# hsinnan75/MapCaller

Hardware: AMD Instinct MI355X
Metric: reads/sec (150 bp PE vs GRCh38) at 1/2/4/8 MI355X; SAM CIGAR bit-exact (higher is better)
Workload: dtype u64/int32; 1 GPU; synthetic GRCh38-sized genome, 3100 Mbp (synthetic: GRCh38 is unavailable offline; repeat landscape in the detail record), 4000000 pairs x 150 bp PE per step per GPU (sub 0.005, ins 0.001, del 0.001 per base), -alg ksw2

## Files before the change

mapcaller_amd/csrc/mcx_glue.h:

```cpp
#ifndef MCX_GLUE_H
#define MCX_GLUE_H
#include "mcx_fm.h"

namespace mcx {

struct Ctx {
    IndexView ix;
    Params pm;
    Caps caps;
    Layout lay;
    uint8_t *detail;
    DetailLayout dlay;
    uint8_t *state;
    const uint8_t *mapq_tab;
    int32_t mapq_rows;
    uint32_t *cig_pool;
    uint32_t *cig_pool_n;
    uint32_t cig_pool_cap;
    const uint32_t *packed;
    int32_t wpad;
    const uint32_t *read_ext;
    int32_t dp_summary;
    const Hit *seed_pool;
};

constexpr int kCigStage = 4;

static inline MCX_HD int64_t hit_pd(const Hit &h) { return h.gPos - h.rPos; }

static inline MCX_HD int prep_seeds(Hit *h, int n)
{
    int m = 0;
    bool in_order = true;
    int64_t ppd = 0;
    int prp = 0;
    for (int i = 0; i < n; i++) {
        const Hit x = h[i];
        const int64_t pd = hit_pd(x);
        if (pd > 0) {
            if (m > 0 && (ppd > pd || (ppd == pd && prp > x.rPos))) in_order = false;
            if (m != i) h[m] = x;
            m++; ppd = pd; prp = x.rPos;
        }
    }
    if (in_order) return m;
    for (int gap = m > 24 ? (m > 400 ? 109 : 23) : 1; gap >= 1; gap = gap > 23 ? 23 : (gap > 5 ? 5 : (gap > 1 ? 1 : 0))) {
        for (int i = gap; i < m; i++) {
            const Hit key = h[i];
            const int64_t kpd = hit_pd(key);
            int j = i - gap;
            while (j >= 0) {
                const Hit y = h[j];
                const int64_t pd = hit_pd(y);
                if (pd > kpd || (pd == kpd && y.rPos > key.rPos)) { h[j + gap] = y; j -= gap; } else break;
            }
            if (j + gap != i) h[j + gap] = key;
        }
    }
    return m;
}

static inline MCX_HD int64_t boundary_of(const IndexView &ix, int64_t gPos)
{
    int s = end_slot(ix, gPos);
    return s < 0 ? -1 : ix.end_pos[s];
}

static inline MCX_HD void cand_init(Cand &dst, int score, int first, int count, int64_t pd0)
{
    Cand c;
    c.score = score; c.mate = -1; c.first = first; c.count = count; c.pd0 = pd0;
    c.frag_off = 0; c.n_frags = 0; c.flag = 0; c.fwd = 1; c.in_pool = 0; c.pad = 0; c.pool_off = 0;
    dst = c;
}

template <class Emit>
static inline MCX_HD int cluster_seeds_to(const IndexView &ix, const Params &pm, int rlen, const Hit *h, int n, Emit emit)
{
    if (n == 0) return 0;
    const Hit h0 = h[0];
    int nc = 0, head = 0, score = h0.len, thr = rlen >> 2;
    int64_t g_end = boundary_of(ix, h0.gPos);
    int64_t pd_prev = hit_pd(h0);
    for (int j = 1; j <= n; j++) {
        Hit hj; hj.gPos = ix.G2; hj.rPos = 0; hj.len = 0;
        if (j < n) hj = h[j];
        const int64_t gj = hj.gPos, pdj = j < n ? hit_pd(hj) : ix.G2;
        int64_t d = pdj - pd_prev;
        pd_prev = pdj;
        if (d < 0) d = -d;
        if (gj > g_end || d > pm.max_pos_diff) {
            if (score > thr) {
                if (thr < (score >> 1)) thr = score >> 1;
                int b = head, e = j, s = score;
                if (score >= rlen) {
                    int run_b = head, rs = h[head].len;
                    s = 0; b = e = head;
                    int k;
                    for (k = head + 1; k < j; k++) {
                        if (hit_pd(h[k]) != hit_pd(h[run_b])) {
                            if (rs > s) { s = rs; b = run_b; e = k; }
                            run_b = k; rs = h[k].len;
                        } else rs += h[k].len;
                    }
                    if (rs > s) { s = rs; b = run_b; e = k; }
                }
                emit(nc, s, b, e - b, hit_pd(h[b]));
                nc++;
            }
            head = j;
            if (j < n) { g_end = boundary_of(ix, gj); score = hj.len; }
        } else score += hj.len;
    }
    return nc;
}

static inline MCX_HD int cluster_seeds(const IndexView &ix, const Params &pm, int rlen, const Hit *h, int n,
                                       Cand *out, int cap)
{
    return cluster_seeds_to(ix, pm, rlen, h, n, [&](int k, int score, int first, int count, int64_t pd0) { if (k < cap) cand_init(out[k], score, first, count, pd0); });
}

static inline MCX_HD void keep_top_scores(Cand *c, int n)
{
    if (n <= 1) return;
    int best = 0;
    for (int i = 0; i < n; i++) if (c[i].score > best) best = c[i].score;
    for (int i = 0; i < n; i++) if (c[i].score < best) c[i].score = 0;
}

static inline MCX_HD int pair_by_distance(int64_t est, Cand *c1, int n1, Cand *c2, int n2, int &lo, int &hi)
{
    int64_t max_lt = -1, min_ge = 0x7fffffff;
    if (n1 * n2 > 100) { keep_top_scores(c1, n1); keep_top_scores(c2, n2); }
    int j0 = 0;
    auto partner = [&](const Cand &a, int &ps) {
        int pick = -1;
        ps = 0;
        while (j0 < n2 && c2[j0].pd0 < a.pd0) j0++;
        for (int j = j0; j < n2; j++) {
            const int sj = c2[j].score;
            if (sj == 0) continue;
            const int64_t d = c2[j].pd0 - a.pd0;
            if (d < est) {
                if (d > max_lt) max_lt = d;
                if (sj > ps) { pick = j; ps = sj; }
            } else { if (d < min_ge) min_ge = d; break; }
        }
        return pick;
    };
    int64_t top = 0;
    for (int i = 0; i < n1; i++) {
        const Cand a = c1[i];
        if (a.score == 0) continue;
        int ps;
        if (partner(a, ps) >= 0) { const int64_t s = (int64_t)a.score + ps; if (s > top) top = s; }
    }
    int paired = 0;
    if (top > 0) {
        j0 = 0;
        for (int i = 0; i < n1; i++) {
            const Cand a = c1[i];
            if (a.score == 0) continue;
            int ps;
            const int pick = partner(a, ps);
            if (pick >= 0 && (int64_t)a.score + ps == top) { paired++; c1[i].mate = pick; c2[pick].mate = i; }
        }
    }
    lo = (int)(max_lt + 1);
    hi = (int)min_ge;
    return paired;
}

static inline MCX_HD void mask_unpaired(Cand *c1, int n1, Cand *c2, int n2)
{
    int top = 0;
    for (int i = 0; i < n1; i++)
        if (c1[i].mate != -1 && top < c1[i].score + c2[c1[i].mate].score) top = c1[i].score + c2[c1[i].mate].score;
    for (int i = 0; i < n1; i++)
        if (c1[i].mate == -1 || c1[i].score + c2[c1[i].mate].score < top) c1[i].score = 0;
    for (int j = 0; j < n2; j++)
        if (c2[j].mate == -1 || c2[j].score + c1[c2[j].mate].score < top) c2[j].score = 0;
}

#define MCX_NOKMER 0xFFFFFFFFu

static inline MCX_HD uint8_t read_char(const ReadRef &r, int i)
{
    if (!r.flipped) return r.ascii[i];
    switch (r.ascii[r.rlen - 1 - i]) {
    case 'A': case 'a': return 'T';
    case 'C': case 'c': return 'G';
    case 'G': case 'g': return 'C';
    case 'T': case 't': return 'A';
    default: return 'N';
    }
}

template <class GetCh>
static inline MCX_HD void kmer_fill(GetCh ch, int len, uint32_t *out)
{
    for (int i = 0; i < len; i++) out[i] = MCX_NOKMER;
    uint32_t tail = 0, count = 0, head, wid;
    while (count < (uint32_t)kKmerSize && tail < (uint32_t)len) { if (ch(tail++) != 'N') count++; else count = 0; }
    if (count != (uint32_t)kKmerSize) return;
    head = tail - kKmerSize;
    wid = 0;
    for (uint32_t i = head; i < head + kKmerSize; i++) wid = (wid << 2) + (uint32_t)nt4_code(ch(i));
    out[head] = wid;
    for (head += 1; tail < (uint32_t)len; head++, tail++) {
        uint8_t c = ch(tail);
        if (c != 'N') {
            wid = ((wid & 0x3FFFu) << 2) + (uint32_t)nt4_code(c);
            out[head] = wid;
        } else {
            count = 0; tail++;
            while (count < (uint32_t)kKmerSize && tail < (uint32_t)len) { if (ch(tail++) != 'N') count++; else count = 0; }
            if (count != (uint32_t)kKmerSize) break;
            head = tail - kKmerSize;
            wid = 0;
            for (uint32_t i = head; i < head + kKmerSize; i++) wid = (wid << 2) + (uint32_t)nt4_code(ch(i));
            out[head] = wid;
        }
    }
}

struct RescueOut { int score; int n_seeds; int d; };

static inline MCX_HD int diag_scan(const uint32_t *kq, int qlen, const uint32_t *kg, int slen, int d, int64_t base,
                                   Hit *hits, int n_hits, int cap, int &emitted, bool &overflow)
{
    const int r0 = d < 0 ? -d : 0, r1 = qlen - 1 < slen - 1 - d ? qlen - 1 : slen - 1 - d;
    int total = 0, run = 0, run_start = 0;
    for (int r = r0; r <= r1 + 1; r++) {
        const bool m = r <= r1 && kq[r] != MCX_NOKMER && kq[r] == kg[r + d];
        if (m) { if (run == 0) run_start = r; run++; }
        else if (run > 0) {
            const int l = kKmerSize + run - 1;
            if (l >= 10) {
                total += l;
                if (hits) {
                    if (n_hits + emitted < cap) {
                        Hit h; h.rPos = run_start; h.gPos = (int64_t)(run_start + d) + base; h.len = l;
                        hits[n_hits + emitted] = h;
                    } else overflow = true;
                    emitted++;
                }
            }
            run = 0;
        }
    }
    return total;
}

static inline MCX_HD int diag_total(const uint32_t *kq, int qlen, const uint32_t *kg, int slen, int d)
{
    const int r0 = d < 0 ? -d : 0, r1 = qlen - 1 < slen - 1 - d ? qlen - 1 : slen - 1 - d;
    int total = 0;
    uint64_t hist = 0;
    for (int base = r0; base <= r1; base += 61) {
        uint64_t e = hist;
        const int n = r1 - base + 1 < 61 ? r1 - base + 1 : 61;
        for (int i = 0; i < n; i++) {
            const uint32_t q = kq[base + i];
            e |= (uint64_t)(q != MCX_NOKMER && q == kg[base + i + d]) << (3 + i);
        }
        const uint64_t t = e & (e >> 1) & (e >> 2);
        const uint64_t own = t & ~(uint64_t)1;
#if defined(__HIP_DEVICE_COMPILE__)
        total += __popcll(own) + 9 * __popcll(own & ~(t << 1));
#else
        total += __builtin_popcountll(own) + 9 * __builtin_popcountll(own & ~(t << 1));
#endif
        hist = (e >> 61) & 7u;
    }
    return total;
}

struct RescueSerial {
    uint32_t *kq, *kg;
    MCX_HD bool leader() const { return true; }
    MCX_HD void sync() const {}
    MCX_HD void fill_query(const ReadRef &rq) const
    {
        kmer_fill([&](uint32_t i) { return read_char(rq, (int)i); }, rq.rlen, kq);
    }
    MCX_HD RescueOut window(const IndexView &ix, int64_t left, int slen, int qlen, Hit *hits, int n_hits, int cap, bool &overflow) const
    {
        kmer_fill([&](uint32_t i) { return (uint8_t)"ACGT"[ref_code(ix, left + i)]; }, slen, kg);
        RescueOut best; best.score = 0; best.n_seeds = 0; best.d = 0;
        int dummy = 0;
        for (int d = -(qlen - 1); d <= slen - 1; d++) {
            const int total = diag_scan(kq, qlen, kg, slen, d, left, nullptr, 0, 0, dummy, overflow);
            if (total > best.score) { best.score = total; best.d = d; }
        }
        if (best.score > 0) diag_scan(kq, qlen, kg, slen, best.d, left, hits, n_hits, cap, best.n_seeds, overflow);
        return best;
    }
};

#if defined(__HIPCC__)
constexpr int kRescueQWords = 1024 / 32 + 2;
constexpr int rescue_wwords(int kg) { return (kg + 2 * 1056) / 32 + 4; }

static __device__ __forceinline__ uint32_t even_bits16(uint32_t t)
{
    t &= 0x55555555u; t = (t | (t >> 1)) & 0x33333333u; t = (t | (t >> 2)) & 0x0f0f0f0fu; t = (t | (t >> 4)) & 0x00ff00ffu;
    return (t | (t >> 8)) & 0xffffu;
}

struct RescueWave {
    uint32_t *q;
    uint32_t *w;
    uint32_t *ew;
    int wstride;
    int *red;
    uint32_t *kq, *kg;
    __device__ bool leader() const { return threadIdx.x == 0; }
    __device__ void sync() const { __threadfence_block(); __syncthreads(); }
    __device__ void fill_query(const ReadRef &rq) const
    {
        const int tid = threadIdx.x, nt = blockDim.x;
        uint32_t *ql = q, *qh = q + kRescueQWords, *qn = q + 2 * kRescueQWords;
        __syncthreads();
        for (int i = tid; i < 3 * kRescueQWords; i += nt) q[i] = 0u;
        if (tid == 0) red[0] = 0;
        __syncthreads();
        for (int i = tid; i < rq.rlen; i += nt) {
            const int c = nt4_code(read_char(rq, i));
            const uint32_t bit = 1u << (i & 31);
            if (c > 3) atomicOr(&qn[i >> 5], bit);
            else { if (c & 1) atomicOr(&ql[i >> 5], bit); if (c & 2) atomicOr(&qh[i >> 5], bit); }
        }
        __syncthreads();
        int any_n = 0;
        for (int k = tid; k < kRescueQWords; k += nt) any_n |= qn[k] != 0u;
        any_n = __syncthreads_or(any_n);
        if (tid == 0) red[2 * (nt >> 6) + 4] = any_n;
        if (any_n) {
            if (leader()) kmer_fill([&](uint32_t i) { return read_char(rq, (int)i); }, rq.rlen, kq);
            __threadfence_block();
            __syncthreads();
            return;
        }
        uint32_t v8 = 0;
        if (tid < kRescueQWords) {
            auto ok = [&](int k) -> uint32_t {
                if (k >= kRescueQWords || 32 * k >= rq.rlen) return 0u;
                const uint32_t in = rq.rlen - 32 * k >= 32 ? ~0u : ((1u << (rq.rlen - 32 * k)) - 1u);
                return ~qn[k] & in;
            };
            const uint32_t v = ok(tid), vn = ok(tid + 1);
            v8 = v;
#pragma unroll
            for (int j = 1; j < kKmerSize; j++) v8 &= __funnelshift_r(v, vn, j);
        }
        __syncthreads();
        if (tid < kRescueQWords) qn[tid] = v8;
        __syncthreads();
    }
    __device__ int diagonal(int d, int qlen, int slen, int pad, bool store) const
    {
        const uint32_t *ql = q, *qh = q + kRescueQWords, *qv = q + 2 * kRescueQWords, *wl = w, *wh = w + wstride;
        const int lo = d < 0 ? -d : 0, hi = qlen - kKmerSize < slen - kKmerSize - d ? qlen - kKmerSize : slen - kKmerSize - d;
        if (hi - lo < 2) return 0;
        const int ktop = (hi + kKmerSize - 1) >> 5, kbot = lo >> 5;
        const int s0 = d + pad, sh = s0 & 31;
        int i = ktop + (s0 >> 5);
        uint32_t wl_hi = wl[i + 1], wh_hi = wh[i + 1], m_hi = 0, a_hi = 0, b_hi = 0, e_hi = 0, t_hi = 0;
        int total = 0;
        for (int k = ktop; k >= kbot; k--, i--) {
            const uint32_t wl_lo = wl[i], wh_lo = wh[i];
            const uint32_t gl = __funnelshift_r(wl_lo, wl_hi, sh), gh = __funnelshift_r(wh_lo, wh_hi, sh);
            wl_hi = wl_lo; wh_hi = wh_lo;
            const uint32_t m = ~((ql[k] ^ gl) | (qh[k] ^ gh));
            const uint32_t a = m & __funnelshift_r(m, m_hi, 1);
            const uint32_t b = a & __funnelshift_r(a, a_hi, 2);
            const uint32_t c = b & __funnelshift_r(b, b_hi, 4);
            m_hi = m; a_hi = a; b_hi = b;
            const int x0 = lo - 32 * k, x1 = hi - 32 * k;
            const uint32_t rows = (x1 < 0 || x0 > 31) ? 0u : ((~0u << (x0 > 0 ? x0 : 0)) & (~0u >> (31 - (x1 < 31 ? x1 : 31))));
            const uint32_t e = c & qv[k] & rows;
            if (store) ew[k] = e;
            uint32_t t = 0;
            if (e | e_hi) {
                t = e & __funnelshift_r(e, e_hi, 1) & __funnelshift_r(e, e_hi, 2);
                total += __popc(t) + 9 * __popc(t & ~__funnelshift_r(t, t_hi, 1));
            }
            t_hi = t; e_hi = e;
        }
        return total;
    }
    __device__ RescueOut window_ids(const IndexView &ix, int64_t left, int slen, int qlen, Hit *hits, int n_hits, int cap, bool &overflow) const
    {
        const int tid = threadIdx.x, nt = blockDim.x, lane = tid & 63, wave = tid >> 6, n_waves = nt >> 6;
        __syncthreads();
        uint8_t *gb = (uint8_t *)(kg + slen + 8);
        if (left < ix.G && left + slen > ix.G) {
            for (int p = tid; p < slen; p += nt) {
                uint32_t wid = MCX_NOKMER;
                if (p + kKmerSize <= slen) { wid = 0; for (int k = 0; k < kKmerSize; k++) wid = (wid << 2) | (uint32_t)ref_code(ix, left + p + k); }
                kg[p] = wid;
            }
        } else {
        const bool rev = left >= ix.G;
        const int64_t f0 = rev ? ix.G2 - (left + slen) : left;
        const int64_t b0 = f0 >> 2;
        const int n_bytes = (int)(((f0 + slen - 1) >> 2) - b0) + 1;
        for (int i = tid; i < n_bytes; i += nt) gb[i] = ix.pac[b0 + i];
        __syncthreads();
        auto base = [&](int p) -> uint32_t {
            const int64_t f = rev ? f0 + (slen - 1 - p) : f0 + p;
            const uint32_t c = (gb[(f >> 2) - b0] >> ((~f & 3) << 1)) & 3u;
            return rev ? 3u - c : c;
        };
        for (int p = tid; p < slen; p += nt) {
            uint32_t wid = MCX_NOKMER;
// ... 891 lines not shown
```

mapcaller_amd/csrc/mcx_pipeline.hip:

```cpp
#include <hip/hip_runtime.h>
#include <algorithm>
#include <atomic>
#include <chrono>
#include <cmath>
#include <cstdio>
#include <cstdlib>
#include <cstring>
#include <string>
#include <type_traits>
#include <vector>

#include "../../include/mcx.h"
#include "mcx_dp.h"
#include "mcx_dp_lane2.h"
#include "mcx_simple.h"
#include "mcx_profile.h"
#include <hipcub/hipcub.hpp>
#include "mcx_internal.h"

using namespace mcx;

static thread_local std::string g_err;
static int fail(int code, const std::string &msg) { g_err = msg; return code; }
#define HIP_TRY(expr)                                                                         \
// ... 581 lines not shown
__global__ void __launch_bounds__(256) k_sa(Ctx cx, SeedOut so, int paired, uint32_t *lf_total)
{
    const uint32_t n = min(*so.n_tasks, so.task_cap);
    const int nr = paired ? 2 : 1;
    for (uint32_t t = blockIdx.x * blockDim.x + threadIdx.x; t < n; t += gridDim.x * blockDim.x) {
        const uint2 task = so.tasks[t];
        PairState st = pair_state(cx.state, cx.lay, cx.caps, task.x / nr);
        Hit &h = st.hits[task.x % nr][task.y];
        int lf = 0;
        h.gPos = (int64_t)fm_sa(cx.ix, (uint64_t)h.gPos, lf);
        if (lf_total && lf) atomicAdd(lf_total, (uint32_t)lf);
    }
}

struct RescueList { uint32_t *ids; uint32_t *n; uint32_t cap; };
struct EarlyList { uint32_t *ids; int32_t *est; uint32_t *n; uint32_t cap; uint32_t *n_hits; };

constexpr int kCntPad = 64;
constexpr int kWorkClasses = 6;
static __device__ __forceinline__ int work_class(uint32_t hits) { return hits > 64 ? 0 : hits > 32 ? 1 : hits > 16 ? 2 : hits > 8 ? 3 : hits > 4 ? 4 : 5; }

static __device__ __forceinline__ int pair_work_class(const PairSel &sel, uint32_t local, const uint32_t *read_blocks, int nr, const uint8_t *done = nullptr)
{
    if (done && done[local]) return -1;
    const uint32_t pair = sel_pair(sel, local);
    return work_class((read_blocks[pair * nr] >> 20) + (nr == 2 ? read_blocks[pair * nr + 1] >> 20 : 0u));
}

constexpr int kOrderTile = 16;

__global__ void __launch_bounds__(256) k_order_count(PairSel sel, const uint32_t *read_blocks, int nr, uint32_t *counts, const uint8_t *done)
{
    __shared__ uint32_t n_cls[kWorkClasses];
    if (threadIdx.x < kWorkClasses) n_cls[threadIdx.x] = 0u;
    __syncthreads();
    const uint32_t base = blockIdx.x * (256u * kOrderTile);
    for (int t = 0; t < kOrderTile; t++) {
        const uint32_t local = base + t * 256u + threadIdx.x;
        const int cls = local < sel.n ? pair_work_class(sel, local, read_blocks, nr, done) : -1;
#pragma unroll
        for (int k = 0; k < kWorkClasses; k++) {
            const uint64_t m = __ballot(cls == k);
            if ((threadIdx.x & 63) == 0 && m) atomicAdd(&n_cls[k], (uint32_t)__popcll(m));
        }
    }
    __syncthreads();
    if (threadIdx.x < kWorkClasses && n_cls[threadIdx.x]) atomicAdd(counts + threadIdx.x * kCntPad, n_cls[threadIdx.x]);
}

__global__ void __launch_bounds__(256) k_order_place(PairSel sel, const uint32_t *read_blocks, int nr, uint32_t *counts, uint32_t *order, const uint8_t *done)
{
    __shared__ uint32_t n_cls[kWorkClasses], at_cls[kWorkClasses];
    if (threadIdx.x < kWorkClasses) n_cls[threadIdx.x] = 0u;
    __syncthreads();
    const uint32_t base = blockIdx.x * (256u * kOrderTile);
    const int lane = threadIdx.x & 63;
    int cls[kOrderTile];
#pragma unroll
    for (int t = 0; t < kOrderTile; t++) {
        const uint32_t local = base + t * 256u + threadIdx.x;
        cls[t] = local < sel.n ? pair_work_class(sel, local, read_blocks, nr, done) : -1;
#pragma unroll
        for (int k = 0; k < kWorkClasses; k++) {
            const uint64_t m = __ballot(cls[t] == k);
            if (lane == 0 && m) atomicAdd(&n_cls[k], (uint32_t)__popcll(m));
        }
    }
    __syncthreads();
    if (threadIdx.x < kWorkClasses) {
        uint32_t first = 0;
        for (int k = 0; k < (int)threadIdx.x; k++) first += counts[k * kCntPad];
        const uint32_t mine = n_cls[threadIdx.x];
        at_cls[threadIdx.x] = first + (mine ? atomicAdd(counts + (8 + threadIdx.x) * kCntPad, mine) : 0u);
    }
    __syncthreads();
#pragma unroll
    for (int t = 0; t < kOrderTile; t++) {
        const uint32_t local = base + t * 256u + threadIdx.x;
#pragma unroll
        for (int k = 0; k < kWorkClasses; k++) {
            const uint64_t m = __ballot(cls[t] == k);
            uint32_t b = 0;
            if (lane == 0 && m) b = atomicAdd(&at_cls[k], (uint32_t)__popcll(m));
            b = __shfl(b, 0, 64);
            if (cls[t] == k) order[b + (uint32_t)__popcll(m & ((1ull << lane) - 1ull))] = local;
        }
    }
}

struct SimpleLater {
    uint32_t *pairs;
    SimpleJob *jobs;
    SimpleRes *res;
    uint32_t *job_list;
    uint32_t *n_pairs, *n_jobs;
    uint32_t cap;
};

template <bool NW, int MODE, bool DETAIL>
__global__ void __launch_bounds__(256) k_simple(Ctx cx, ReadBatch rb, uint32_t n_pairs, const int32_t *est, const uint32_t *read_blocks, AlnRec *recs, PairOut *pout,
                                                uint8_t *done, uint32_t *pool_over, uint32_t *n_done, SimpleLater sl)
{
    __shared__ EndsLds ends;
    __shared__ uint16_t cig_stage[256 * 2 * kSimpleRuns];
    __shared__ uint32_t job_stage[MODE == kDpCollect ? 3 * kSimpleJobs * 256 : 1];
    stage_ends(cx.ix, ends);
    const uint32_t slot = blockIdx.x * blockDim.x + threadIdx.x;
    const int nr = cx.pm.paired ? 2 : 1;
    uint16_t *stage = cig_stage + threadIdx.x;
    const uint32_t n_slots = MODE == kDpReplay ? min(*sl.n_pairs, sl.cap) : n_pairs;
    bool ok = slot < n_slots;
    const uint32_t pair = MODE == kDpReplay ? (ok ? sl.pairs[slot] : 0u) : slot;
    SimpleRead sr[2];
    int rl[2] = {0, 0};
    typename std::conditional<DETAIL, SimpleDetail, SimpleNoDetail>::type det;
    SimpleDpIo io;
    io.mode = MODE == kDpCollect && !sl.pairs ? kDpNone : MODE;
    io.jobs = MODE == kDpCollect ? job_stage + threadIdx.x : nullptr; io.job_stride = 256;
    io.res = MODE == kDpReplay ? sl.res + (uint64_t)slot * kSimpleJobs : nullptr;
    io.n = 0; io.read = 0;
    bool later = false;
    if (ok) {
        const PairState st = pair_state(cx.state, cx.lay, cx.caps, pair);
#pragma unroll
        for (int s = 0; s < 2; s++) {
            if (s < nr && ok) {
                const uint32_t r = pair * nr + s;
                const int nh = (int)(read_blocks[r] >> 20);
                rl[s] = (int)(rb.off[r + 1] - rb.off[r]);
                io.read = r;
                ok = nh >= 1 && nh <= kSimpleHits && !(cx.read_ext[r] >> 31);
                if (ok) {
                    if constexpr (DETAIL) { uint8_t *rec = cx.detail + (uint64_t)r * cx.dlay.stride; det.frags = (Frag *)(rec + sizeof(DetailHdr)); det.ops = rec + cx.dlay.off_ops; }
                    const int how = simple_read<NW, uint16_t>(cx.ix, cx.pm, rl[s], cx.packed + (uint64_t)r * cx.wpad, st.hits[s], nh, sr[s], stage + s * kSimpleRuns * 256, 256, io, det);
                    ok = how != kSimpleNo;
                    later = later || how == kSimpleLater;
                }
            }
        }
        if (ok && nr == 2) ok = simple_pair_ok(sr[0], sr[1], est[pair]);
    }
    if (MODE == kDpCollect) {
        const bool wait = ok && later;
        const uint32_t at = wave_reserve(sl.n_pairs, wait ? 1u : 0u);
        const bool kept = wait && at < sl.cap;
        const uint32_t jat = wave_reserve(sl.n_jobs, kept ? (uint32_t)io.n : 0u);
        if (kept) {
            sl.pairs[at] = pair;
            for (int k = 0; k < io.n; k++) {
                const uint32_t *w = job_stage + (3 * k) * 256 + threadIdx.x;
                sl.jobs[(uint64_t)at * kSimpleJobs + k] = simple_job_unpack(w[0], w[256], w[512], pair * (uint32_t)nr, nr);
                sl.job_list[jat + k] = at * kSimpleJobs + (uint32_t)k;
            }
            done[pair] = 2;
        }
        if (wait) ok = false;
        later = kept;
    }
    const uint32_t want = ok ? (uint32_t)sr[0].n_cig + (nr == 2 ? (uint32_t)sr[1].n_cig : 0u) : 0u;
    const uint32_t at = wave_reserve(cx.cig_pool_n, want);
    const uint64_t took = __ballot(ok);
    if ((threadIdx.x & 63) == 0 && took) atomicAdd(n_done, (uint32_t)__popcll(took));
    if (slot >= n_slots) return;
    if (ok && at + want > cx.cig_pool_cap) { atomicOr(pool_over, 1u); ok = false; }
    if (!later) done[pair] = ok ? 1 : 0;
    if (!ok) return;
    const uint32_t off[2] = {at, at + (uint32_t)sr[0].n_cig};
#pragma unroll
    for (int s = 0; s < 2; s++) {
        if (s >= nr) break;
        for (int k = 0; k < sr[s].n_cig; k++) cx.cig_pool[off[s] + k] = (uint32_t)stage[(s * kSimpleRuns + k) * 256];
    }
    AlnRec rec2[2];
    PairOut po;
    simple_pair(cx, nr == 2, sr[0], sr[nr - 1], rl[0], rl[nr - 1], est[pair], rec2, off, po);
    recs[(uint64_t)pair * nr] = rec2[0];
    if (nr == 2) recs[(uint64_t)pair * nr + 1] = rec2[1];
    pout[pair] = po;
    if constexpr (DETAIL) {
#pragma unroll
        for (int s = 0; s < 2; s++) {
            if (s >= nr) break;
            const DetailHdr d = simple_detail_hdr(cx.ix, nr == 2, s, sr[0], sr[nr - 1]);
            *(DetailHdr *)(cx.detail + ((uint64_t)pair * nr + s) * cx.dlay.stride) = d;
        }
    }
}

template <bool NW>
__global__ void __launch_bounds__(256) k_simple_dp(Ctx cx, SimpleLater sl)
{
    constexpr int W = 2 + kSimpleDp * LaneDir<16, NW>::words;
    __shared__ uint32_t words[W * 256];
    const uint32_t n = min(*sl.n_jobs, sl.cap * kSimpleJobs);
    LaneMem mem; mem.base = words; mem.stride = 256; mem.lane = threadIdx.x;
    for (uint32_t i = blockIdx.x * blockDim.x + threadIdx.x; i < n; i += gridDim.x * blockDim.x) {
        const uint32_t at = sl.job_list[i];
        const SimpleJob j = sl.jobs[at];
        sl.res[at] = simple_dp_job<NW>(cx.ix, j, cx.packed + (uint64_t)j.read * cx.wpad, mem);
    }
}

static __device__ __forceinline__ uint32_t listed_pairs(const PairSel &sel, const uint32_t *order_cnt)
{
    if (!order_cnt) return sel.n;
    uint32_t n = 0;
#pragma unroll
    for (int k = 0; k < kWorkClasses; k++) n += order_cnt[k * kCntPad];
    return n;
}

__global__ void __launch_bounds__(256) k_cluster(Ctx cx, ReadBatch rb, PairSel sel, RescueList rl, const uint32_t *read_blocks, EarlyList el, const uint32_t *order,
                                                 const uint32_t *order_cnt, int cls_lo, int cls_hi)
{
    __shared__ EndsLds ends;
    uint32_t first = 0, n_listed = listed_pairs(sel, order_cnt);
    if (order_cnt && order) {
        uint32_t at = 0;
        for (int k = 0; k < kWorkClasses; k++) { if (k == cls_lo) first = at; at += order_cnt[k * kCntPad]; if (k == cls_hi) n_listed = at; }
    }
    if (first + blockIdx.x * blockDim.x >= n_listed) return;
    stage_ends(cx.ix, ends);
    const uint32_t slot = first + blockIdx.x * blockDim.x + threadIdx.x;
    const bool in = slot < n_listed;
    const uint32_t local = in ? (order ? order[slot] : slot) : 0u;
    uint32_t need = 0, over = 0;
    if (in) {
        ReadRef rd[2];
        make_reads(cx, rb, sel_pair(sel, local), rd);
        PairState st = pair_state(cx.state, cx.lay, cx.caps, local);
        const uint32_t pair = sel_pair(sel, local);
        const int nr = cx.pm.paired ? 2 : 1;
        int nh[2] = {(int)(read_blocks[pair * nr] >> 20), nr == 2 ? (int)(read_blocks[pair * nr + 1] >> 20) : 0};
        stage_cluster_pair(cx, local, rd, sel.est[local], nh);
        const uint32_t fl = st.hdr->flags;
        need = (cx.pm.paired && !(fl & kOvAny) && st.hdr->n_paired == 0) ? 1u : 0u;
        over = (el.ids && (fl & kOvAny)) ? 1u : 0u;
        if (over && (fl & kOvHits)) atomicAdd(el.n_hits, 1u);
        if (over) st.hdr->flags = fl | kDispatched;
        else if (need) st.hdr->flags = fl | kAwaitRescue;
    }
    const uint32_t at = wave_reserve(rl.n, need);
    if (need && at < rl.cap) rl.ids[at] = local;
    if (el.ids) {
        const uint32_t ea = wave_reserve(el.n, over);
        if (over && ea < el.cap) { el.ids[ea] = sel_pair(sel, local); el.est[ea] = sel.est[local]; }
    }
}

__global__ void k_publish_early(const uint32_t *n, const uint32_t *any_n, volatile uint32_t *host)
{
    if (threadIdx.x == 0) { host[0] = *n; host[1] = *any_n; __threadfence_system(); }
}

struct ClusterLds {
    Hit *hits;
    int64_t *pd[2];
    int32_t *score[2];
    uint32_t *span[2];
    int32_t *mate[2];
    int32_t *pick;
};

static inline MCX_HD int cluster_sort_room(int hit_cap) { int p = 1; while (p < hit_cap) p <<= 1; return p; }
static inline size_t cluster_lds_bytes(int hit_cap, int cand_cap) { return (size_t)cluster_sort_room(hit_cap) * sizeof(Hit) + (size_t)cand_cap * (2 * (8 + 4 + 4 + 4) + 4) + 64; }
constexpr int kClusterSmall = 192;

__global__ void __launch_bounds__(64) k_cluster_wave(Ctx cx, ReadBatch rb, PairSel sel, RescueList rl, const uint32_t *read_blocks, int hits_lo, int hits_hi, int lds_hits,
                                                     int lds_cands)
{
    extern __shared__ __attribute__((aligned(16))) uint8_t cl_lds[];
    __shared__ EndsLds ends;
    stage_ends(cx.ix, ends);
    const int lane = threadIdx.x;
    const int nr = cx.pm.paired ? 2 : 1;
    ClusterLds L;
    {
        uint8_t *p = cl_lds;
        L.hits = (Hit *)p; p += (size_t)cluster_sort_room(lds_hits) * sizeof(Hit);
        for (int s = 0; s < 2; s++) { L.pd[s] = (int64_t *)p; p += (size_t)lds_cands * 8; }
        for (int s = 0; s < 2; s++) { L.score[s] = (int32_t *)p; p += (size_t)lds_cands * 4; }
        for (int s = 0; s < 2; s++) { L.span[s] = (uint32_t *)p; p += (size_t)lds_cands * 4; }
        for (int s = 0; s < 2; s++) { L.mate[s] = (int32_t *)p; p += (size_t)lds_cands * 4; }
        L.pick = (int32_t *)p;
    }
    auto wave_sync = [] { __builtin_amdgcn_fence(__ATOMIC_SEQ_CST, "workgroup"); __builtin_amdgcn_s_barrier(); };
    for (uint32_t local = blockIdx.x; local < sel.n; local += gridDim.x) {
        const uint32_t pair = sel_pair(sel, local);
        {
            const int h0 = (int)(read_blocks[pair * nr] >> 20), h1 = nr == 2 ? (int)(read_blocks[pair * nr + 1] >> 20) : 0, hm = h0 > h1 ? h0 : h1;
            if (hm <= hits_lo || hm > hits_hi) continue;
        }
        PairState st = pair_state(cx.state, cx.lay, cx.caps, local);
        uint32_t flags = 0;
        int n_hits[2] = {0, 0}, n_cands[2] = {0, 0};
        for (int s = 0; s < nr; s++) {
            const uint32_t r = pair * nr + s;
            const int rlen = (int)(rb.off[r + 1] - rb.off[r]);
            int nh = (int)(read_blocks[r] >> 20);
            if (nh > cx.caps.hit_seed) { flags |= kOvHits; nh = 0; }
            Hit *g_hits = st.hits[s];
            wave_sync();
            int m = 0;
            for (int base = 0; base < nh; base += 64) {
                const int i = base + lane;
                Hit x; x.gPos = 0; x.rPos = 0; x.len = 0;
                bool keep = false;
                if (i < nh) { x = g_hits[i]; keep = hit_pd(x) > 0; }
                const uint64_t mask = __ballot(keep);
                if (keep) L.hits[m + __popcll(mask & ((1ull << lane) - 1ull))] = x;
                m += __popcll(mask);
            }
            int P = 1;
            while (P < m) P <<= 1;
            for (int i = m + lane; i < P; i += 64) { Hit x; x.gPos = (int64_t)1 << 62; x.rPos = 0; x.len = 0; L.hits[i] = x; }
            wave_sync();
            for (int k = 2; k <= P; k <<= 1)
                for (int j = k >> 1; j > 0; j >>= 1) {
                    for (int i = lane; i < P; i += 64) {
                        const int o = i ^ j;
                        if (o > i) {
                            const Hit a = L.hits[i], b = L.hits[o];
                            const int64_t pa = hit_pd(a), pb = hit_pd(b);
                            const bool a_gt = pa > pb || (pa == pb && a.rPos > b.rPos);
                            if (((i & k) == 0) == a_gt) { L.hits[i] = b; L.hits[o] = a; }
                        }
                    }
                    wave_sync();
                }
            for (int i = lane; i < m; i += 64) g_hits[i] = L.hits[i];
            int nc = 0;
            if (lane == 0)
                nc = cluster_seeds_to(cx.ix, cx.pm, rlen, L.hits, m, [&](int k, int score, int first, int count, int64_t pd0) {
                    if (k < cx.caps.cand_seed) { L.pd[s][k] = pd0; L.score[s][k] = score; L.span[s][k] = (uint32_t)first | ((uint32_t)count << 16); }
                });
            nc = __shfl(nc, 0, 64);
            if (nc > cx.caps.cand_seed) { flags |= kOvCands; nc = 0; }
            n_hits[s] = m; n_cands[s] = nc;
            wave_sync();
        }
        for (int s = 0; s < 2; s++) for (int i = lane; i < n_cands[s]; i += 64) L.mate[s][i] = -1;
        wave_sync();
        int n_paired = 0, lo = 0, hi = 0x7fffffff;
        if (cx.pm.paired && !(flags & kOvAny)) {
            const int n1 = n_cands[0], n2 = n_cands[1];
            const int64_t est = (int64_t)sel.est[local];
            if (n1 * n2 > 100)
                for (int s = 0; s < 2; s++) {
                    int best = 0;
                    for (int i = lane; i < n_cands[s]; i += 64) best = max(best, L.score[s][i]);
                    for (int o = 32; o > 0; o >>= 1) best = max(best, __shfl_xor(best, o, 64));
                    if (n_cands[s] > 1) for (int i = lane; i < n_cands[s]; i += 64) if (L.score[s][i] < best) L.score[s][i] = 0;
                }
            wave_sync();
            int64_t max_lt = -1, min_ge = 0x7fffffff, top = 0;
            for (int i = lane; i < n1; i += 64) {
                const int sa = L.score[0][i];
                const int64_t pa = L.pd[0][i];
                int pick = -1, ps = 0;
                if (sa != 0)
                    for (int j = 0; j < n2; j++) {
                        const int sj = L.score[1][j];
                        const int64_t pj = L.pd[1][j];
                        if (sj == 0 || pj < pa) continue;
                        const int64_t d = pj - pa;
                        if (d < est) { if (d > max_lt) max_lt = d; if (sj > ps) { pick = j; ps = sj; } }
                        else if (d < min_ge) min_ge = d;
                    }
                L.pick[i] = pick;
                if (pick >= 0 && (int64_t)sa + ps > top) top = (int64_t)sa + ps;
            }
            for (int o = 32; o > 0; o >>= 1) {
                const int64_t a = __shfl_xor(max_lt, o, 64), b = __shfl_xor(min_ge, o, 64), c = __shfl_xor(top, o, 64);
                if (a > max_lt) max_lt = a;
                if (b < min_ge) min_ge = b;
                if (c > top) top = c;
            }
            wave_sync();
            if (top > 0)
                for (int i = lane; i < n1; i += 64) {
                    const int pick = L.pick[i];
                    if (pick >= 0 && (int64_t)L.score[0][i] + L.score[1][pick] == top) {
                        n_paired++;
                        L.mate[0][i] = pick;
                        atomicMax(&L.mate[1][pick], i);
                    }
                }
            for (int o = 32; o > 0; o >>= 1) n_paired += __shfl_xor(n_paired, o, 64);
            lo = (int)(max_lt + 1); hi = (int)min_ge;
            wave_sync();
        }
        for (int s = 0; s < nr; s++)
            for (int i = lane; i < n_cands[s]; i += 64) {
                Cand c;
                c.score = L.score[s][i]; c.mate = (int16_t)L.mate[s][i]; c.first = (int16_t)(L.span[s][i] & 0xFFFFu); c.count = (int16_t)(L.span[s][i] >> 16); c.pd0 = L.pd[s][i];
                c.frag_off = 0; c.n_frags = 0; c.flag = 0; c.fwd = 1; c.in_pool = 0; c.pad = 0; c.pool_off = 0;
                st.cands[s][i] = c;
            }
        if (lane == 0) {
            PairHdr h;
            h.flags = flags; h.n_frags = 0; h.n_ops = 0; h.pair_dist = 0; h.n_jobs = 0; h.pair_ok = 0; h.mapped = 0; h.pad[0] = h.pad[1] = 0;
            h.n_hits[0] = (int16_t)n_hits[0]; h.n_hits[1] = (int16_t)n_hits[1]; h.n_cands[0] = (int16_t)n_cands[0]; h.n_cands[1] = (int16_t)n_cands[1];
            h.sum[0].best = h.sum[1].best = -1; h.sum[0].score = h.sum[1].score = 0; h.sum[0].sub = h.sum[1].sub = 0;
            h.est = sel.est[local]; h.est_lo = lo; h.est_hi = hi; h.n_paired = (int16_t)n_paired;
            if (cx.pm.paired && !(flags & kOvAny) && n_paired == 0) h.flags |= kAwaitRescue;
            *st.hdr = h;
            if (cx.pm.paired && !(flags & kOvAny) && n_paired == 0) {
                const uint32_t at = atomicAdd(rl.n, 1u);
                if (at < rl.cap) rl.ids[at] = local;
            }
        }
    }
}

constexpr int kRescueThreads = 256;
constexpr unsigned kRescueBlocks = 4096;
constexpr size_t kRescueScratchWords = 1024 + (4096 + 64 + 8) + (4096 + 64) / 16 + 8;

template <int KG>
#ifndef MCX_RESCUE_WAVES
#define MCX_RESCUE_WAVES 1
#endif
__global__ void __launch_bounds__(kRescueThreads, MCX_RESCUE_WAVES) k_rescue(Ctx cx, ReadBatch rb, PairSel sel, RescueList rl, uint32_t *kscratch)
{
    __shared__ uint32_t q[3 * kRescueQWords];
    __shared__ uint32_t w[2 * rescue_wwords(KG)];
    __shared__ uint32_t ew[kRescueQWords];
    __shared__ int red[2 * (kRescueThreads / 64) + 5];
    const uint32_t n = min(*rl.n, rl.cap);
    RescueWave ev; ev.q = q; ev.w = w; ev.ew = ew; ev.wstride = rescue_wwords(KG); ev.red = red;
    ev.kq = kscratch + (size_t)blockIdx.x * kRescueScratchWords; ev.kg = ev.kq + 1024;
    for (uint32_t i = blockIdx.x; i < n; i += gridDim.x) {
        const uint32_t local = rl.ids[i];
        ReadRef rd[2];
        make_reads(cx, rb, sel_pair(sel, local), rd);
        stage_rescue(cx, local, rd, ev);
        __syncthreads();
    }
}

struct RescueTask {
    uint32_t local;
    uint16_t side, ci;
    int32_t slen, sb;
    int64_t left;
    int32_t pad[2];
};
static_assert(sizeof(RescueTask) == 32, "RescueTask is two 16-byte records");
struct RescueRes { int32_t score, d, n_seeds; uint32_t seed_off; };
struct RescuePlan { uint32_t local, first, n, flags; };

struct RescueWork {
    RescueTask *tasks; RescueRes *res; Hit *seeds; RescuePlan *plans;
    uint32_t *n_tasks, *n_plans, *n_seeds;
    uint32_t task_cap, seed_cap;
    uint32_t *ids_n, *n_ids_n;
};

__global__ void __launch_bounds__(256) k_rescue_plan(Ctx cx, ReadBatch rb, PairSel sel, RescueList rl, RescueWork rw)
{
    __shared__ EndsLds ends;
    stage_ends(cx.ix, ends);
    const IndexView &ix = cx.ix;
    const uint32_t n = min(*rl.n, rl.cap);
    for (uint32_t i = blockIdx.x * blockDim.x + threadIdx.x; i < n; i += gridDim.x * blockDim.x) {
        const uint32_t local = rl.ids[i];
        const uint32_t pair = sel_pair(sel, local);
        PairState st = pair_state(cx.state, cx.lay, cx.caps, local);
        const PairHdr h = *st.hdr;
        if ((h.flags & kOvAny) || h.n_paired != 0) continue;
        if ((cx.read_ext[2 * pair] | cx.read_ext[2 * pair + 1]) >> 31) {
            const uint32_t at = atomicAdd(rw.n_ids_n, 1u);
            rw.ids_n[at] = local;
            continue;
        }
        const int rlen[2] = {(int)(rb.off[2 * pair + 1] - rb.off[2 * pair]), (int)(rb.off[2 * pair + 2] - rb.off[2 * pair + 1])};
        const int n1 = h.n_cands[0], n2 = h.n_cands[1];
        const Cand *c1 = st.cands[0], *c2 = st.cands[1];
        int s1 = 0, s2 = 0;
        for (int k = 0; k < n1; k++) { const int sc = c1[k].score; if (sc > s1) s1 = sc; }
        for (int k = 0; k < n2; k++) { const int sc = c2[k].score; if (sc > s2) s2 = sc; }
        int mode;
        if (s1 < (rlen[0] >> 2) && s2 < (rlen[1] >> 2)) continue;
        else if (s1 - s2 > (rlen[1] >> 2)) mode = 1;
        else if (s2 - s1 > (rlen[0] >> 2)) mode = 2;
        else mode = 3;
        uint32_t flags = kRescueUsedEst;
        const int64_t est = (int64_t)(uint32_t)h.est;
        uint32_t first = 0, count = 0;
        for (int pass = 0; pass < 2; pass++) {
            uint32_t at = first;
            for (int side = 0; side < 2; side++) {
                if (side == 0 && !(mode == 1 || mode == 3)) continue;
                if (side == 1 && !(mode == 2 || mode == 3)) continue;
                const int qlen = side == 0 ? rlen[1] : rlen[0];
                const Cand *ca = side == 0 ? c1 : c2;
                const int na = side == 0 ? n1 : n2, sa = side == 0 ? s1 : s2, sb = side == 0 ? s2 : s1;
                const int thr = sa >> 1;
                for (int ci = 0; ci < na; ci++) {
                    const Cand c = ca[ci];
                    if (c.score < thr || c.mate != -1) continue;
                    const int64_t left = side == 0 ? c.pd0 : c.pd0 - est;
                    int64_t right = side == 0 ? c.pd0 + est + qlen : c.pd0 + qlen;
                    if (right > ix.G2) right = ix.G2;
                    if (left < 0 || right >= ix.G2) continue;
                    const int e1 = end_slot(ix, left), e2 = end_slot(ix, right);
                    if (e1 < 0 || e2 < 0 || ix.end_chr[e1] != ix.end_chr[e2]) continue;
                    const int slen = (int)(right - left);
                    if (slen < qlen) continue;
                    if (slen > cx.caps.kmer_cap) { flags |= kOvKmer; continue; }
                    if (pass == 0) count++;
                    else {
                        if (at < rw.task_cap) {
                            RescueTask t; t.local = local; t.side = (uint16_t)side; t.ci = (uint16_t)ci; t.slen = slen; t.sb = sb; t.left = left; t.pad[0] = t.pad[1] = 0;
                            rw.tasks[at] = t;
                        }
                        at++;
                    }
                }
            }
            if (pass == 0) first = count ? atomicAdd(rw.n_tasks, count) : 0u;
        }
        RescuePlan pl; pl.local = local; pl.first = first; pl.n = count; pl.flags = flags;
        rw.plans[atomicAdd(rw.n_plans, 1u)] = pl;
    }
}

template <int KG>
__global__ void __launch_bounds__(256) k_rescue_eval(Ctx cx, ReadBatch rb, PairSel sel, RescueWork rw)
{
    constexpr int kWaves = 4, kW = rescue_wwords(KG);
    __shared__ uint32_t q_all[kWaves][3 * kRescueQWords];
    __shared__ uint32_t w_all[kWaves][2 * kW];
    __shared__ uint32_t ew_all[kWaves][kRescueQWords];
    __shared__ uint16_t ss_all[kWaves][128];
    const IndexView &ix = cx.ix;
    const int lane = threadIdx.x & 63, wv = threadIdx.x >> 6;
    RescueWave ev; ev.q = q_all[wv]; ev.w = w_all[wv]; ev.ew = ew_all[wv]; ev.wstride = kW; ev.red = nullptr; ev.kq = ev.kg = nullptr;
    uint32_t *ql = ev.q, *qh = ev.q + kRescueQWords, *qv = ev.q + 2 * kRescueQWords, *wl = ev.w, *wh = ev.w + kW;
    const uint32_t n = min(*rw.n_tasks, rw.task_cap);
    auto wave_sync = [] { __builtin_amdgcn_fence(__ATOMIC_SEQ_CST, "wavefront"); __builtin_amdgcn_wave_barrier(); };
    for (uint32_t t = blockIdx.x * kWaves + wv; t < n; t += gridDim.x * kWaves) {
        const RescueTask task = rw.tasks[t];
        const uint32_t pair = sel_pair(sel, task.local), r = 2 * pair + (task.side == 0 ? 1u : 0u);
        const int qlen = (int)(rb.off[r + 1] - rb.off[r]), slen = task.slen;
        const uint32_t *codes = cx.packed + (uint64_t)r * cx.wpad;
        wave_sync();
        for (int k = lane; k < kRescueQWords; k += 64) {
            uint32_t lo = 0, hi = 0, in = 0;
            if (32 * k < qlen) {
                const uint32_t a = codes[2 * k], b = 32 * k + 16 < qlen ? codes[2 * k + 1] : 0u;
                lo = (__brev(even_bits16(a)) >> 16) | (__brev(even_bits16(b)) & 0xFFFF0000u);
                hi = (__brev(even_bits16(a >> 1)) >> 16) | (__brev(even_bits16(b >> 1)) & 0xFFFF0000u);
                in = qlen - 32 * k >= 32 ? ~0u : ((1u << (qlen - 32 * k)) - 1u);
                lo &= in; hi &= in;
            }
            ql[k] = lo; qh[k] = hi; qv[k] = in;
        }
        wave_sync();
        uint32_t v8 = 0;
        if (lane < kRescueQWords) {
            const uint32_t v = qv[lane], vn = lane + 1 < kRescueQWords ? qv[lane + 1] : 0u;
            v8 = v;
#pragma unroll
            for (int j = 1; j < kKmerSize; j++) v8 &= __funnelshift_r(v, vn, j);
        }
        wave_sync();
        if (lane < kRescueQWords) qv[lane] = v8;
        const int pad = ((qlen + 31) & ~31) + 32;
        const int n_words = (pad + slen + qlen) / 32 + 3;
        for (int j = lane; j < n_words; j += 64) {
            uint32_t lo = 0, hi = 0;
            const int p0 = 32 * j - pad;
            if (p0 >= 0 && p0 < slen) {
#pragma unroll
                for (int half = 0; half < 2; half++) {
                    const int p = p0 + 16 * half;
                    if (p >= slen) break;
                    const uint32_t x = ref_codes16(ix, task.left + p);
                    uint32_t l16 = __brev(even_bits16(x)) >> 16, h16 = __brev(even_bits16(x >> 1)) >> 16;
                    if (slen - p < 16) { const uint32_t keep = (1u << (slen - p)) - 1u; l16 &= keep; h16 &= keep; }
                    lo |= l16 << (16 * half); hi |= h16 << (16 * half);
                }
            }
            wl[j] = lo; wh[j] = hi;
        }
        wave_sync();
        const int d_lo = -(qlen - kKmerSize - 2), n_diag = slen - kKmerSize - 2 - d_lo + 1;
        uint32_t key = 0;
        for (int g = lane; g < n_diag; g += 64) {
            const int total = ev.diagonal(d_lo + g, qlen, slen, pad, false);
            const uint32_t k2 = ((uint32_t)total << 13) | (uint32_t)(8191 - g);
            if (total > 0 && k2 > key) key = k2;
        }
#pragma unroll
        for (int o = 32; o > 0; o >>= 1) { const uint32_t other = (uint32_t)__shfl_xor((int)key, o, 64); if (other > key) key = other; }
        RescueRes res; res.score = (int)(key >> 13); res.d = 0; res.n_seeds = 0; res.seed_off = 0;
        if (key != 0) {
            res.d = d_lo + (8191 - (int)(key & 8191u));
            if (res.score > task.sb) {
                for (int k = lane; k < kRescueQWords; k += 64) ev.ew[k] = 0u;
                wave_sync();
                if (lane == 0) ev.diagonal(res.d, qlen, slen, pad, true);
                wave_sync();
                uint32_t S = 0, E = 0;
                if (lane < kRescueQWords) {
                    const uint32_t e0 = ev.ew[lane], e1 = lane + 1 < kRescueQWords ? ev.ew[lane + 1] : 0u, ep = lane > 0 ? ev.ew[lane - 1] : 0u;
                    const uint32_t t = e0 & __funnelshift_r(e0, e1, 1) & __funnelshift_r(e0, e1, 2);
                    const uint32_t t_before = (ep >> 31) & e0 & (e0 >> 1) & 1u;
                    const uint32_t t_after = e1 & (e1 >> 1) & (e1 >> 2) & 1u;
                    S = t & ~((t << 1) | t_before);
                    E = t & ~((t >> 1) | (t_after << 31));
                }
                const int cs = __popc(S), ce = __popc(E);
                int is = cs, ie = ce;
#pragma unroll
                for (int o = 1; o < 64; o <<= 1) {
                    const int vs = __shfl_up(is, o, 64), ve = __shfl_up(ie, o, 64);
                    if (lane >= o) { is += vs; ie += ve; }
                }
                const int n_seeds = __shfl(is, 63, 64);
                uint32_t off = 0;
                if (lane == 0) off = atomicAdd(rw.n_seeds, (uint32_t)n_seeds);
                off = (uint32_t)__shfl((int)off, 0, 64);
                res.n_seeds = n_seeds; res.seed_off = off;
                if ((uint64_t)off + (uint64_t)n_seeds <= rw.seed_cap) {
                    uint16_t *ss = ss_all[wv];
                    int j = is - cs;
                    for (uint32_t m = S; m; m &= m - 1u) ss[j++] = (uint16_t)(32 * lane + __ffs((int)m) - 1);
                    wave_sync();
                    Hit *out = rw.seeds + off;
                    j = ie - ce;
                    for (uint32_t m = E; m; m &= m - 1u, j++) {
                        const int start = ss[j], end = 32 * lane + __ffs((int)m) - 1;
                        Hit h; h.rPos = start; h.gPos = (int64_t)(start + res.d) + task.left; h.len = end - start + 1 + kKmerSize + 1;
                        out[j] = h;
                    }
                }
            }
// ... 2993 lines not shown
```

Baseline: 534.2 million reads/s.

## Parallelize seed clustering across the wavefront with prefix scans for single-contig reads

When all kept hits of a read fall within one contig, the serial lane-0 clustering loop is replaced by a wave-wide scan. Lanes find cluster heads and tails, compute cluster scores with prefix sums, apply the running-max keep threshold with prefix max, and emit candidates in order via ballot compaction. This is meant to remove the single-lane serial bottleneck in clustering. It adds several shuffle scans per 64-hit chunk, and the output must match the serial version for candidate order and thresholds to stay bit-exact.

```diff
diff --git a/mapcaller_amd/csrc/mcx_glue.h b/mapcaller_amd/csrc/mcx_glue.h
--- a/mapcaller_amd/csrc/mcx_glue.h
+++ b/mapcaller_amd/csrc/mcx_glue.h
@@ -113,6 +113,46 @@
         } else score += hj.len;
     }
     return nc;
+}
+
+static inline MCX_HD bool clu_one_contig(const IndexView &ix, int64_t g_min, int64_t g_max)
+{
+    const int s = end_slot(ix, g_min);
+    return s >= 0 && s == end_slot(ix, g_max);
+}
+
+static inline MCX_HD bool clu_head(const Params &pm, const Hit *h, int j)
+{
+    if (j == 0) return true;
+    int64_t d = hit_pd(h[j]) - hit_pd(h[j - 1]);
+    if (d < 0) d = -d;
+    return d > pm.max_pos_diff;
+}
+
+static inline MCX_HD bool clu_keep(int rlen, int score, int prev_max)
+{
+    const int thr = (rlen >> 2) > (prev_max >> 1) ? (rlen >> 2) : (prev_max >> 1);
+    return score > thr;
+}
+
+template <class Emit>
+static inline MCX_HD void clu_emit(int rlen, const Hit *h, int b, int e, int score, int k, Emit emit)
+{
+    int s = score;
+    if (score >= rlen) {
+        const int head = b, j = e;
+        int run_b = head, rs = h[head].len;
+        s = 0; b = e = head;
+        int i;
+        for (i = head + 1; i < j; i++) {
+            if (hit_pd(h[i]) != hit_pd(h[run_b])) {
+                if (rs > s) { s = rs; b = run_b; e = i; }
+                run_b = i; rs = h[i].len;
+            } else rs += h[i].len;
+        }
+        if (rs > s) { s = rs; b = run_b; e = i; }
+    }
+    emit(k, s, b, e - b, hit_pd(h[b]));
 }
 
 static inline MCX_HD int cluster_seeds(const IndexView &ix, const Params &pm, int rlen, const Hit *h, int n,
diff --git a/mapcaller_amd/csrc/mcx_pipeline.hip b/mapcaller_amd/csrc/mcx_pipeline.hip
--- a/mapcaller_amd/csrc/mcx_pipeline.hip
+++ b/mapcaller_amd/csrc/mcx_pipeline.hip
@@ -907,15 +907,20 @@
             Hit *g_hits = st.hits[s];
             wave_sync();
             int m = 0;
+            int64_t g_min = INT64_MAX, g_max = INT64_MIN;
             for (int base = 0; base < nh; base += 64) {
                 const int i = base + lane;
                 Hit x; x.gPos = 0; x.rPos = 0; x.len = 0;
                 bool keep = false;
                 if (i < nh) { x = g_hits[i]; keep = hit_pd(x) > 0; }
                 const uint64_t mask = __ballot(keep);
-                if (keep) L.hits[m + __popcll(mask & ((1ull << lane) - 1ull))] = x;
+                if (keep) {
+                    L.hits[m + __popcll(mask & ((1ull << lane) - 1ull))] = x;
+                    g_min = min(g_min, x.gPos); g_max = max(g_max, x.gPos);
+                }
                 m += __popcll(mask);
             }
+            for (int o = 32; o > 0; o >>= 1) { g_min = min(g_min, __shfl_xor(g_min, o, 64)); g_max = max(g_max, __shfl_xor(g_max, o, 64)); }
             int P = 1;
             while (P < m) P <<= 1;
             for (int i = m + lane; i < P; i += 64) { Hit x; x.gPos = (int64_t)1 << 62; x.rPos = 0; x.len = 0; L.hits[i] = x; }
@@ -934,12 +939,39 @@
                     wave_sync();
                 }
             for (int i = lane; i < m; i += 64) g_hits[i] = L.hits[i];
+            auto to_lds = [&](int k, int score, int first, int count, int64_t pd0) {
+                if (k < cx.caps.cand_seed) { L.pd[s][k] = pd0; L.score[s][k] = score; L.span[s][k] = (uint32_t)first | ((uint32_t)count << 16); }
+            };
             int nc = 0;
-            if (lane == 0)
-                nc = cluster_seeds_to(cx.ix, cx.pm, rlen, L.hits, m, [&](int k, int score, int first, int count, int64_t pd0) {
-                    if (k < cx.caps.cand_seed) { L.pd[s][k] = pd0; L.score[s][k] = score; L.span[s][k] = (uint32_t)first | ((uint32_t)count << 16); }
-                });
-            nc = __shfl(nc, 0, 64);
+            if (m == 0) {
+            } else if (clu_one_contig(cx.ix, g_min, g_max)) {
+                int c_len = 0, c_head = 0, c_hlen = 0, c_max = 0;
+                auto scan_add = [&](int v) { for (int o = 1; o < 64; o <<= 1) { const int t = __shfl_up(v, o, 64); if (lane >= o) v += t; } return v; };
+                auto scan_max = [&](int v) { for (int o = 1; o < 64; o <<= 1) { const int t = __shfl_up(v, o, 64); if (lane >= o && t > v) v = t; } return v; };
+                for (int base = 0; base < m; base += 64) {
+                    const int j = base + lane;
+                    const bool in = j < m;
+                    const int len = in ? L.hits[j].len : 0;
+                    const bool head = in && clu_head(cx.pm, L.hits, j);
+                    const bool tail = in && (j == m - 1 || clu_head(cx.pm, L.hits, j + 1));
+                    const int incl = c_len + scan_add(len);
+                    int hj = scan_max(head ? j : -1), hl = scan_max(head ? incl - len : -1);
+                    if (hj < 0) { hj = c_head; hl = c_hlen; }
+                    const int score = incl - hl;
+                    const int tmax = scan_max(tail ? score : 0);
+                    int prev = __shfl_up(tmax, 1, 64);
+                    prev = lane == 0 ? c_max : max(prev, c_max);
+                    const bool keep = tail && clu_keep(rlen, score, prev);
+                    const uint64_t km = __ballot(keep);
+                    if (keep) clu_emit(rlen, L.hits, hj, j + 1, score, nc + __popcll(km & ((1ull << lane) - 1ull)), to_lds);
+                    nc += __popcll(km);
+                    c_len = __shfl(incl, 63, 64); c_head = __shfl(hj, 63, 64); c_hlen = __shfl(hl, 63, 64);
+                    c_max = max(c_max, __shfl(tmax, 63, 64));
+                }
+            } else {
+                if (lane == 0) nc = cluster_seeds_to(cx.ix, cx.pm, rlen, L.hits, m, to_lds);
+                nc = __shfl(nc, 0, 64);
+            }
             if (nc > cx.caps.cand_seed) { flags |= kOvCands; nc = 0; }
             n_hits[s] = m; n_cands[s] = nc;
             wave_sync();
```

After: 533.8 million reads/s (median of 3 runs). No clear change (-0.1%).
